# intel/intel-extension-for-transformers

Measured on AMD Instinct MI355X. Metric: decode tokens/sec + achieved HBM GB/s, Llama-2-7B int4 WOQ, batch=1, higher is better.
Workload: dtype int4 weights x fp32 activations (3 int8 limbs on i8 MFMA, exact int32 tile sums, fp32 across tiles); 1 GPU; Llama-2-7B int4 sym group_size=128 fp16 scales, batch=1 greedy decode, prompt 32, lm_head fp16 unquantised, KV fp16; global_batch=1, parallelism=single GPU, hipgraph=True

## Files before the change

intel_extension_for_transformers_amd/csrc/woq_ops.hip:

```cpp
#include "woq_attn_decode.h"
#include "woq_device.h"
#include "woq_host.h"
#include "woq_xq.h"
#include "../../include/woq_hip_experimental.h"

namespace woq {

__global__ __launch_bounds__(256) void rmsnorm_kernel(const void* __restrict__ x, int dtype,
                                                      const float* __restrict__ w, float eps, int d,
                                                      void* __restrict__ out, int out_dtype) {
  __shared__ float part[4];
  const size_t row = blockIdx.x;
  const int tid = threadIdx.x;
  float ss = 0.f;
  for (int i = tid; i < d; i += 256) {
    float v = load_f32(x, row * d + i, dtype);
    ss = fmaf(v, v, ss);
  }
  ss = wave_sum(ss);
  if ((tid & 63) == 0) part[tid >> 6] = ss;
  __syncthreads();
  const float tot = part[0] + part[1] + part[2] + part[3];
  const float inv = 1.0f / sqrtf(tot / (float)d + eps);
  for (int i = tid; i < d; i += 256) {
    float v = load_f32(x, row * d + i, dtype);
    store_f32(out, row * d + i, out_dtype, v * inv * w[i]);
  }
}

__global__ void rope_kernel(void* __restrict__ x, int dtype, const int32_t* __restrict__ pos,
                            const float* __restrict__ cs, const float* __restrict__ sn, int heads, int D,
                            size_t total_pairs) {
  size_t idx = (size_t)blockIdx.x * blockDim.x + threadIdx.x;
  if (idx >= total_pairs) return;
  const int half = D >> 1;
  const int i = (int)(idx % half);
  const size_t th = idx / half;
  const int t = (int)(th / heads);
  const int p = pos[t];
  const float c = cs[(size_t)p * half + i], s = sn[(size_t)p * half + i];
  const size_t base = th * D;
  const float a = load_f32(x, base + i, dtype), b = load_f32(x, base + i + half, dtype);
  store_f32(x, base + i, dtype, a * c - b * s);
  store_f32(x, base + i + half, dtype, b * c + a * s);
}

__global__ void silu_mul_kernel(const void* __restrict__ g, const void* __restrict__ u, int dtype, size_t n,
                                void* __restrict__ out) {
  size_t idx = (size_t)blockIdx.x * blockDim.x + threadIdx.x;
  const size_t stride = (size_t)gridDim.x * blockDim.x;
  for (; idx < n; idx += stride) {
    const float a = load_f32(g, idx, dtype), b = load_f32(u, idx, dtype);
    store_f32(out, idx, dtype, a / (1.0f + expf(-a)) * b);
  }
}

__global__ void gelu_kernel(const void* __restrict__ x, int dtype, size_t n, int approximate,
                            void* __restrict__ out) {
  size_t idx = (size_t)blockIdx.x * blockDim.x + threadIdx.x;
  const size_t stride = (size_t)gridDim.x * blockDim.x;
  for (; idx < n; idx += stride) {
    const float v = load_f32(x, idx, dtype);
    float r;
    if (approximate)
      r = 0.5f * v * (1.0f + tanhf(0.7978845608028654f * (v + 0.044715f * v * v * v)));
    else
      r = 0.5f * v * (1.0f + erff(v * 0.7071067811865476f));
    store_f32(out, idx, dtype, r);
  }
}


__global__ void embed_kernel(const void* __restrict__ embed, int dtype, const int32_t* __restrict__ token, int hidden,
                             float* __restrict__ out, const float* __restrict__ norm_w, XqPtrs xo,
                             float* __restrict__ ssq_out, unsigned int* __restrict__ step_seq,
                             int32_t* __restrict__ pos, int max_ctx, int* __restrict__ status) {
  const int i = blockIdx.x * blockDim.x + threadIdx.x;
  if (i == 0) {
    if (step_seq != nullptr) step_seq[0] = step_seq[0] + 1u;
    if (pos != nullptr && pos[0] >= max_ctx) {
      pos[0] = max_ctx - 1;
      if (status != nullptr) atomicOr(status, 2);
    }
  }
  if (i < hidden) {
    const float v = load_f32(embed, (size_t)token[0] * hidden + i, dtype);
    out[i] = v;
    if (xo.limbs != nullptr) {
      const float ss = row16_sum(v * v);
      if ((i & 15) == 0) ssq_out[i >> 4] = ss;
      xq_emit16(v * norm_w[i], xo, i >> 4, i & 15);
    }
  }
}

__global__ __launch_bounds__(256) void argmax_embed_kernel(const float* __restrict__ pmax, const int32_t* __restrict__ pidx,
                                                           int n_pairs, int32_t* __restrict__ token,
                                                           int32_t* __restrict__ pos, int32_t* __restrict__ log,
                                                           const void* __restrict__ embed, int dtype, int hidden,
                                                           float* __restrict__ out, const float* __restrict__ norm_w,
                                                           XqPtrs xo, float* __restrict__ ssq_out,
                                                           unsigned int* __restrict__ step_seq, int max_ctx,
                                                           int* __restrict__ status) {
  __shared__ float bv[4];
  __shared__ int bi[4];
  const int tid = threadIdx.x, lane = tid & 63, wid = tid >> 6;
  float best = -INFINITY;
  int idx = 0x7fffffff;
  for (int i = tid; i < n_pairs; i += 256) {
    const float v = pmax[i];
    const int ci = pidx[i];
    if (v > best || (v == best && ci < idx)) best = v, idx = ci;
  }
#pragma unroll
  for (int o = 32; o > 0; o >>= 1) {
    const float ov = __shfl_xor(best, o, 64);
    const int oi = __shfl_xor(idx, o, 64);
    if (ov > best || (ov == best && oi < idx)) best = ov, idx = oi;
  }
  if (lane == 0) bv[wid] = best, bi[wid] = idx;
  __syncthreads();
  best = bv[0], idx = bi[0];
#pragma unroll
  for (int w = 1; w < 4; ++w)
    if (bv[w] > best || (bv[w] == best && bi[w] < idx)) best = bv[w], idx = bi[w];
  const bool no_winner = idx < 0 || (size_t)idx >= (size_t)n_pairs * 16;
  if (no_winner) idx = 0;
  if (blockIdx.x == 0 && tid == 0) {
    if (no_winner && status != nullptr) atomicOr(status, 4);
    token[0] = idx;
    int p = pos[0];
    if (log != nullptr) log[p] = idx;
    p += 1;
    if (step_seq != nullptr) step_seq[0] = step_seq[0] + 1u;
    if (p >= max_ctx) {
      p = max_ctx - 1;
      if (status != nullptr) atomicOr(status, 2);
    }
    pos[0] = p;
  }
  const int i = blockIdx.x * 256 + tid;
  if (i < hidden) {
    const float v = load_f32(embed, (size_t)idx * hidden + i, dtype);
    out[i] = v;
    if (xo.limbs != nullptr) {
      const float ss = row16_sum(v * v);
      if ((i & 15) == 0) ssq_out[i >> 4] = ss;
      xq_emit16(v * norm_w[i], xo, i >> 4, i & 15);
    }
  }
}

template <typename KV, int HD, bool SPLIT>
__global__ __launch_bounds__(256) void attn_decode_kernel(const float* __restrict__ qkv, KV* __restrict__ kcache,
                                                          KV* __restrict__ vcache, const int32_t* __restrict__ pos_p,
                                                          const float* __restrict__ cs, const float* __restrict__ sn,
                                                          int hk, int window, int spw,
                                                          float* __restrict__ out, XqPtrs xo, AttnMerge mg) {
  extern __shared__ __attribute__((aligned(16))) float sm[];
  const int heads = hk & 0xffff, kv_heads = hk >> 16;
  const int bx = (int)blockIdx.x;
  const int h = (heads & 7) == 0 ? (bx & 7) * (heads >> 3) + (bx >> 3) : bx;
  attn_decode_body<KV, HD, SPLIT>(sm, h, (int)blockIdx.y, (int)gridDim.y, AttnPlain{qkv}, kcache, vcache, pos_p, cs,
                                  sn, heads, kv_heads, window, spw, out, xo);
  if constexpr (SPLIT) {
    if (mg.counter != nullptr) attn_slices_merge<HD, 1>(out, heads, h, 1, (int)gridDim.y, mg.counter + h, mg, sm);
  }
}

template <int HD>
__global__ __launch_bounds__(256) void attn_combine_kernel(const float* __restrict__ part, int ns,
                                                          float* __restrict__ out, XqPtrs xo) {
  __shared__ float ms[64], wl[64], wsc[64], red[256];
  constexpr int GROUPS = 256 / HD;
  constexpr int PER = ATTN_MAX_SLICES / GROUPS;
  const int h = blockIdx.x, tid = threadIdx.x;
  const int d = tid % HD, grp = tid / HD;
  const float* p = part + (size_t)h * ATTN_MAX_SLICES * HD;
  const float* pml = part + (size_t)gridDim.x * ATTN_MAX_SLICES * HD + (size_t)h * ATTN_MAX_SLICES * 2;
  const int si = min(tid, ns - 1);
  const float m_r = pml[si * 2], l_r = pml[si * 2 + 1];
  float v[PER];
#pragma unroll
  for (int u = 0; u < PER; ++u) v[u] = p[(size_t)min(grp + u * GROUPS, ns - 1) * HD + d];
  if (tid < ns) ms[tid] = m_r, wl[tid] = l_r;
  __syncthreads();
  float m = -INFINITY;
  for (int s = 0; s < ns; ++s) m = fmaxf(m, ms[s]);
  if (tid < ns) {
    const float w = ms[tid] == -INFINITY ? 0.f : __expf(ms[tid] - m);
    wsc[tid] = w;
    wl[tid] *= w;
  }
  __syncthreads();
  float l = 0.f;
  for (int s = 0; s < ns; ++s) l += wl[s];
  float o = 0.f;
#pragma unroll
  for (int u = 0; u < PER; ++u) {
    const int s = grp + u * GROUPS;
    if (s < ns) o = fmaf(v[u], wsc[s], o);
  }
  red[tid] = o;
  __syncthreads();
  if (grp == 0) {
    float t = 0.f;
#pragma unroll
    for (int g2 = 0; g2 < GROUPS; ++g2) t += red[g2 * HD + d];
    out[(size_t)h * HD + d] = t / l;
    if (xo.limbs != nullptr) xq_emit16(t / l, xo, (h * HD + d) >> 4, d & 15);
  }
}

__global__ __launch_bounds__(256) void lm_head_kernel(const float* __restrict__ hidden_in,
                                                      const float* __restrict__ norm_w, float eps,
                                                      const void* __restrict__ W, int w_dtype, int hidden, int vocab,
                                                      float* __restrict__ logits, float* __restrict__ pmax,
                                                      int32_t* __restrict__ pidx) {
  extern __shared__ __attribute__((aligned(16))) float sm[];
  float* xs = sm;
  __shared__ float part[4];
  __shared__ float bestv[4];
  __shared__ int besti[4];
  const int tid = threadIdx.x, lane = tid & 63, wid = tid >> 6;
  float wbest = -INFINITY;
  int wbi = 0x7fffffff;
  typedef unsigned int u32x4 __attribute__((ext_vector_type(4)));
  float ss = 0.f;
  for (int i = tid; i < hidden; i += 256) {
    const float v = hidden_in[i];
    xs[i] = v;
    ss = fmaf(v, v, ss);
  }
  ss = wave_sum(ss);
  if (lane == 0) part[wid] = ss;
  __syncthreads();
  const float inv = 1.0f / sqrtf((part[0] + part[1] + part[2] + part[3]) / (float)hidden + eps);
  for (int i = tid; i < hidden; i += 256) xs[i] = xs[i] * inv * norm_w[i];
  __syncthreads();
  const int rows_per_wg = 16;
  auto consume = [&](const u32x4& raw, int k0, float& acc) {
    const uint32_t rr[4] = {raw.x, raw.y, raw.z, raw.w};
#pragma unroll
    for (int j = 0; j < 4; ++j) {
      float lo, hi;
      if (w_dtype == WOQ_BF16) {
        lo = bf16_bits_to_f32(rr[j] & 0xffff);
        hi = bf16_bits_to_f32(rr[j] >> 16);
      } else {
        lo = f16_bits_to_f32(rr[j] & 0xffff);
        hi = f16_bits_to_f32(rr[j] >> 16);
      }
      acc = fmaf(lo, xs[k0 + 2 * j], acc);
      acc = fmaf(hi, xs[k0 + 2 * j + 1], acc);
    }
  };
  auto finish = [&](int v, float acc) {
    acc = wave_sum(acc);
    if (lane == 0) logits[v] = acc;
    if (acc > wbest) {
      wbest = acc;
      wbi = v;
    }
  };
  for (int r = wid; r < rows_per_wg; r += 4) {
    const int v = blockIdx.x * rows_per_wg + r;
    if (v >= vocab) break;
    const uint16_t* wr = (const uint16_t*)W + (size_t)v * hidden;
    float acc = 0.f;
    for (int k0 = lane * 8; k0 < hidden; k0 += 512) consume(__builtin_nontemporal_load((const u32x4*)(wr + k0)), k0, acc);
    finish(v, acc);
  }
  if (pmax) {
    if (lane == 0) {
      bestv[wid] = wbest;
      besti[wid] = wbi;
    }
    __syncthreads();
    if (tid == 0) {
      float b = bestv[0];
      int bi = besti[0];
      for (int w = 1; w < 4; ++w)
        if (bestv[w] > b || (bestv[w] == b && besti[w] < bi)) {
          b = bestv[w];
          bi = besti[w];
        }
      pmax[blockIdx.x] = b;
      pidx[blockIdx.x] = bi;
    }
  }
}

__global__ __launch_bounds__(1024) void argmax_kernel(const float* __restrict__ logits, const int32_t* __restrict__ cand,
                                                      int vocab, int32_t* __restrict__ token,
                                                      int32_t* __restrict__ pos, int32_t* __restrict__ log) {
  __shared__ float bv[16];
  __shared__ int bi[16];
  const int tid = threadIdx.x, lane = tid & 63, wid = tid >> 6;
  float best = -INFINITY;
  int idx = 0x7fffffff;
  for (int i = tid; i < vocab; i += 1024) {
    const float v = logits[i];
    const int ci = cand ? cand[i] : i;
    if (v > best || (v == best && ci < idx)) {
      best = v;
      idx = ci;
    }
  }
#pragma unroll
  for (int o = 32; o > 0; o >>= 1) {
    const float ov = __shfl_xor(best, o, 64);
    const int oi = __shfl_xor(idx, o, 64);
    if (ov > best || (ov == best && oi < idx)) {
      best = ov;
      idx = oi;
    }
  }
  if (lane == 0) {
    bv[wid] = best;
    bi[wid] = idx;
  }
  __syncthreads();
  if (tid == 0) {
    for (int w = 1; w < 16; ++w)
      if (bv[w] > best || (bv[w] == best && bi[w] < idx)) {
        best = bv[w];
        idx = bi[w];
      }
    token[0] = idx;
    if (log != nullptr) log[pos[0]] = idx;
    pos[0] = pos[0] + 1;
  }
}

void launch_embed(const void* embed, int dtype, const int32_t* token, int hidden, float* out, const float* norm_w,
                  const XqPtrs& xo, float* ssq_out, unsigned int* step_seq, int32_t* pos, int max_ctx, int* status,
                  hipStream_t st) {
  hipLaunchKernelGGL(embed_kernel, dim3((hidden + 255) / 256), dim3(256), 0, st, embed, dtype, token, hidden, out,
                     norm_w, xo, ssq_out, step_seq, pos, max_ctx, status);
}

template <typename KV, int HD>
static int launch_attn_t(const float* qkv, void* kcache, void* vcache, const int32_t* pos, const float* cs,
                         const float* sn, int heads, int kv_heads, int max_ctx, int window, float* out, int splits,
                         float* part, const XqPtrs& xo, unsigned int* merge_counters, hipStream_t st) {
  const int reach = window > 0 ? min(window, max_ctx) : max_ctx;
  const int span = splits > 1 ? ((((reach + splits - 1) / splits) + 63) & ~63) + 64 : reach;
  const int spw = attn_dec_spw(span);
  const size_t lds = attn_dec_lds_floats(HD, span) * 4;
  if (lds > 160 * 1024) return woq::fail("QBits: max_ctx too large for the decode attention (raise attn_splits)");
  if (splits > 1) {
    auto k = attn_decode_kernel<KV, HD, true>;
    static bool once = false;
    if (!once) {
      hipFuncSetAttribute((const void*)k, hipFuncAttributeMaxDynamicSharedMemorySize, 160 * 1024);
      once = true;
    }
    const AttnMerge mg{merge_counters, out, xo};
    hipLaunchKernelGGL(k, dim3(heads, splits), dim3(256), lds, st, qkv, (KV*)kcache, (KV*)vcache, pos, cs, sn,
                       heads | (kv_heads << 16), window, spw, part, XqPtrs{nullptr, nullptr, nullptr}, mg);
    if (merge_counters == nullptr)
      hipLaunchKernelGGL(attn_combine_kernel<HD>, dim3(heads), dim3(256), 0, st, part, splits, out, xo);
    return 0;
  }
  auto k = attn_decode_kernel<KV, HD, false>;
  static bool once = false;
  if (!once) {
    hipFuncSetAttribute((const void*)k, hipFuncAttributeMaxDynamicSharedMemorySize, 160 * 1024);
    once = true;
  }
  hipLaunchKernelGGL(k, dim3(heads), dim3(256), lds, st, qkv, (KV*)kcache, (KV*)vcache, pos, cs, sn,
                     heads | (kv_heads << 16), window, spw, out, xo,
                     AttnMerge{nullptr, nullptr, XqPtrs{nullptr, nullptr, nullptr}});
  return 0;
}

int launch_attn_decode(const float* qkv, void* kcache, void* vcache, int kv_dtype, const int32_t* pos,
                       const float* cs, const float* sn, int heads, int kv_heads, int D, int max_ctx, int window,
                       float* out, int splits, int grouped, float* part, const XqPtrs& xo, hipStream_t st,
                       unsigned int* merge_counters, int chunk_fixed, const AttnA2A* a2a_grouped, const unsigned int* seq,
                       int layer) {
  if (D != 64 && D != 128) return woq::fail("QBits: attention head_dim must be 64 or 128");
  if (splits > ATTN_MAX_SLICES) return woq::fail("QBits: at most 64 context slices");
  AttnMerge mg{merge_counters, out, xo};
  const bool a2a = grouped && a2a_grouped != nullptr && merge_counters == nullptr && splits <= 32;
  if (a2a) mg.part_g = a2a_grouped->part_g, mg.seq = seq, mg.layer = layer, mg.status = a2a_grouped->status;
  if (grouped && launch_attn_decode_mfma(qkv, kcache, vcache, kv_dtype, pos, cs, sn, heads, kv_heads, D, window, splits,
                                          part, chunk_fixed, max_ctx, mg, st)) {
    if (merge_counters == nullptr && !a2a) launch_attn_combine(part, heads, D, splits, out, xo, st);
    return 0;
  }
#define WOQ_ATTN_DEC(T)                                                                                              \
  return D == 128 ? launch_attn_t<T, 128>(qkv, kcache, vcache, pos, cs, sn, heads, kv_heads, max_ctx, window, out,   \
                                          splits, part, xo, merge_counters, st)                                     \
                  : launch_attn_t<T, 64>(qkv, kcache, vcache, pos, cs, sn, heads, kv_heads, max_ctx, window, out,    \
                                         splits, part, xo, merge_counters, st);
  if (kv_dtype == WOQ_F16) { WOQ_ATTN_DEC(_Float16) }
  if (kv_dtype == WOQ_FP8_E4M3) { WOQ_ATTN_DEC(Fp8) }
  WOQ_ATTN_DEC(__bf16)
#undef WOQ_ATTN_DEC
}

void launch_attn_combine(const float* part, int heads, int D, int splits, float* out, const XqPtrs& xo,
                         hipStream_t st) {
  if (D == 128)
    hipLaunchKernelGGL(attn_combine_kernel<128>, dim3(heads), dim3(256), 0, st, part, splits, out, xo);
  else
    hipLaunchKernelGGL(attn_combine_kernel<64>, dim3(heads), dim3(256), 0, st, part, splits, out, xo);
}

void launch_lm_head(const float* hidden_in, const float* norm_w, float eps, const void* W, int w_dtype, int hidden,
                    int vocab, float* logits, float* pmax, int32_t* pidx, hipStream_t st) {
  hipLaunchKernelGGL(lm_head_kernel, dim3((vocab + 15) / 16), dim3(256), (size_t)hidden * 4, st, hidden_in, norm_w,
                     eps, W, w_dtype, hidden, vocab, logits, pmax, pidx);
}

void launch_argmax(const float* logits, int vocab, int32_t* token, int32_t* pos, hipStream_t st) {
  hipLaunchKernelGGL(argmax_kernel, dim3(1), dim3(1024), 0, st, logits, (const int32_t*)nullptr, vocab, token, pos,
                     (int32_t*)nullptr);
}

void launch_argmax_pairs(const float* pmax, const int32_t* pidx, int n, int32_t* token, int32_t* pos, int32_t* log,
                         hipStream_t st) {
  hipLaunchKernelGGL(argmax_kernel, dim3(1), dim3(1024), 0, st, pmax, pidx, n, token, pos, log);
}

void launch_argmax_embed(const float* pmax, const int32_t* pidx, int n, int32_t* token, int32_t* pos, int32_t* log,
                         const void* embed, int dtype, int hidden, float* out, const float* norm_w, const XqPtrs& xo,
                         float* ssq_out, unsigned int* step_seq, int max_ctx, int* status, hipStream_t st) {
  hipLaunchKernelGGL(argmax_embed_kernel, dim3((hidden + 255) / 256), dim3(256), 0, st, pmax, pidx, n, token, pos, log,
                     embed, dtype, hidden, out, norm_w, xo, ssq_out, step_seq, max_ctx, status);
}

}

using namespace woq;

extern "C" {

int woq_rmsnorm(const void* x_dev, int dtype, const float* weight_dev, float eps, int rows, int d, void* out_dev,
                int out_dtype, void* stream) {
  WOQ_TRY
  WOQ_CHECK(rows >= 0 && d > 0, "QBits: bad rmsnorm shape");
  if (rows == 0) return 0;
  hipLaunchKernelGGL(rmsnorm_kernel, dim3(rows), dim3(256), 0, (hipStream_t)stream, x_dev, dtype, weight_dev, eps, d,
                     out_dev, out_dtype);
  WOQ_HIP(hipGetLastError());
  WOQ_END
}

int woq_rope(void* x_dev, int dtype, const int32_t* pos_dev, const float* cos_dev, const float* sin_dev, int tokens,
             int heads, int D, void* stream) {
  WOQ_TRY
  WOQ_CHECK((D & 1) == 0, "QBits: rope head_dim must be even");
  size_t total = (size_t)tokens * heads * (D / 2);
  if (total == 0) return 0;
  hipLaunchKernelGGL(rope_kernel, dim3((unsigned)((total + 255) / 256)), dim3(256), 0, (hipStream_t)stream, x_dev,
                     dtype, pos_dev, cos_dev, sin_dev, heads, D, total);
  WOQ_HIP(hipGetLastError());
  WOQ_END
}

int woq_silu_mul(const void* gate_dev, const void* up_dev, int dtype, size_t n, void* out_dev, void* stream) {
  WOQ_TRY
  if (n == 0) return 0;
  unsigned blocks = (unsigned)std::min<size_t>((n + 255) / 256, 2048);
  hipLaunchKernelGGL(silu_mul_kernel, dim3(blocks), dim3(256), 0, (hipStream_t)stream, gate_dev, up_dev, dtype, n,
                     out_dev);
  WOQ_HIP(hipGetLastError());
  WOQ_END
}

int woq_gelu(const void* x_dev, int dtype, size_t n, int approximate, void* out_dev, void* stream) {
  WOQ_TRY
  if (n == 0) return 0;
  unsigned blocks = (unsigned)std::min<size_t>((n + 255) / 256, 2048);
  hipLaunchKernelGGL(gelu_kernel, dim3(blocks), dim3(256), 0, (hipStream_t)stream, x_dev, dtype, n, approximate,
                     out_dev);
  WOQ_HIP(hipGetLastError());
  WOQ_END
}

WOQ_API int woq_probe_attn_decode(const float* qkv, void* kcache, void* vcache, int kv_dtype, const int32_t* pos_dev,
                                  const float* cos_dev, const float* sin_dev, int heads, int kv_heads, int head_dim,
                                  int max_ctx, int window, int splits, int grouped, int merge, int chunk_fixed,
                                  float* out, void* stream) {
  WOQ_TRY
  WOQ_CHECK(heads > 0 && kv_heads > 0 && heads % kv_heads == 0 && max_ctx > 0 && window >= 0 && splits >= 1,
            "QBits: bad attention shape");
  WOQ_CHECK(merge == 0 || merge == 1, "QBits: merge must be 0 (combine launch) or 1 (last-arriver counters)");
  const hipStream_t st = (hipStream_t)stream;
  const size_t part_bytes = (size_t)heads * ATTN_MAX_SLICES * (head_dim + 2) * sizeof(float);
  float* part = nullptr;
  unsigned int* counters = nullptr;
  WOQ_HIP(hipMallocAsync((void**)&part, part_bytes, st));
  if (merge) {
    if (hipMallocAsync((void**)&counters, (size_t)heads * sizeof(unsigned int), st) != hipSuccess ||
        hipMemsetAsync(counters, 0, (size_t)heads * sizeof(unsigned int), st) != hipSuccess) {
      if (counters) hipFreeAsync(counters, st);
      hipFreeAsync(part, st);
      return woq::fail("QBits: could not allocate the attention merge counters");
    }
  }
  const int rc = launch_attn_decode(qkv, kcache, vcache, kv_dtype, pos_dev, cos_dev, sin_dev, heads, kv_heads, head_dim,
                                    max_ctx, window, out, splits, grouped, part, XqPtrs{nullptr, nullptr, nullptr}, st,
                                    counters, chunk_fixed, nullptr, nullptr, 0);
  const hipError_t le = hipGetLastError();
  if (counters) hipFreeAsync(counters, st);
  hipFreeAsync(part, st);
  if (rc) return rc;
  WOQ_HIP(le);
  WOQ_END
}

}
```

Before: 689.4 tokens/s.

## Software-pipeline lm_head weight streaming with buffer loads and templated chunk count

New measurement: 692.9 tokens/s (median of 6 runs). About the same (+0.5%).

```diff
diff --git a/intel_extension_for_transformers_amd/csrc/woq_lm_head.h b/intel_extension_for_transformers_amd/csrc/woq_lm_head.h
--- /dev/null
+++ b/intel_extension_for_transformers_amd/csrc/woq_lm_head.h
@@ -0,0 +1,192 @@
+#pragma once
+#include "woq_device.h"
+#include "woq_gemv_common.h"
+
+namespace woq {
+
+constexpr int LM_WINDOW = 8;
+constexpr int LM_EARLY = 0;
+
+template <bool BF, int CPR, int D, int EARLY>
+__device__ __forceinline__ void lm_head_stream(float* __restrict__ xs, float* __restrict__ part,
+                                               float* __restrict__ bestv, int* __restrict__ besti,
+                                               const float* __restrict__ hidden_in, const float* __restrict__ norm_w,
+                                               float eps, const void* __restrict__ W, int hidden, int vocab,
+                                               float* __restrict__ logits, float* __restrict__ pmax,
+                                               int32_t* __restrict__ pidx) {
+  const int tid = threadIdx.x, lane = tid & 63;
+  const int wid = __builtin_amdgcn_readfirstlane(tid >> 6);
+  const int row0 = (int)blockIdx.x * 16;
+  const int cpr = CPR > 0 ? CPR : (hidden + 511) >> 9;
+  const int total = 4 * cpr;
+  const int pitch = hidden * 2;
+  const rsrc_t rw = make_rsrc((const uint16_t*)W + (size_t)row0 * hidden, min(16, vocab - row0) * pitch);
+  const int lane8 = lane * 8;
+
+  int q_i = 0, q_off = wid * pitch;
+  int c_i = 0, c_row = row0 + wid;
+  u32x4 w[D];
+  auto request = [&](u32x4& dst) {
+    const int k0 = lane8 + (q_i << 9);
+    dst = __builtin_amdgcn_raw_buffer_load_b128(rw, k0 < hidden ? q_off + k0 * 2 : 0x7ffffff0, 0, AUX_NT);
+    if (++q_i == cpr) q_i = 0, q_off += 4 * pitch;
+  };
+  int q_base = wid * pitch + lane8 * 2;
+  auto request_at = [&](u32x4& dst, int c) {
+    const int i = c % cpr;
+    const int off = q_base + ((i & 3) << 10);
+    const bool live = i + 1 < cpr || lane8 + (i << 9) < hidden;
+    dst = __builtin_amdgcn_raw_buffer_load_b128(rw, live ? off : 0x7ffffff0, 0, AUX_NT);
+    if (i + 1 == cpr)
+      q_base += 4 * pitch - ((i >> 2) << 12);
+    else if ((i & 3) == 3)
+      q_base += 4096;
+    else
+      return;
+    asm volatile("" : "+v"(q_base));
+  };
+  auto fill = [&]() {
+#pragma unroll
+    for (int s = 0; s < D; ++s) {
+      if constexpr (CPR > 0) {
+        if (s < 4 * CPR) request_at(w[s], s);
+      } else {
+        if (s < total) request(w[s]);
+      }
+    }
+    __builtin_amdgcn_sched_barrier(0);
+  };
+
+  if constexpr (EARLY == 1) fill();
+  const rsrc_t rh = make_rsrc(hidden_in, hidden * 4), rn = make_rsrc(norm_w, hidden * 4);
+  float ss = 0.f;
+  for (int b = tid; b < hidden; b += 2048) {
+    float v[8];
+#pragma unroll
+    for (int u = 0; u < 8; ++u)
+      v[u] = __builtin_bit_cast(float, __builtin_amdgcn_raw_buffer_load_b32(rh, (b + 256 * u) * 4, 0, 0));
+#pragma unroll
+    for (int u = 0; u < 8; ++u)
+      if (b + 256 * u < hidden) {
+        xs[b + 256 * u] = v[u];
+        ss = fmaf(v[u], v[u], ss);
+      }
+  }
+  if constexpr (EARLY == 2) fill();
+  ss = wave_sum(ss);
+  if (lane == 0) part[wid] = ss;
+  __syncthreads();
+  const float inv = 1.0f / sqrtf((part[0] + part[1] + part[2] + part[3]) / (float)hidden + eps);
+  for (int b = tid; b < hidden; b += 2048) {
+    float g[8];
+#pragma unroll
+    for (int u = 0; u < 8; ++u)
+      g[u] = __builtin_bit_cast(float, __builtin_amdgcn_raw_buffer_load_b32(rn, (b + 256 * u) * 4, 0, 0));
+#pragma unroll
+    for (int u = 0; u < 8; ++u)
+      if (b + 256 * u < hidden) xs[b + 256 * u] = xs[b + 256 * u] * inv * g[u];
+  }
+  __syncthreads();
+  if constexpr (EARLY == 0) fill();
+
+  float wbest = -INFINITY;
+  int wbi = 0x7fffffff;
+  float acc = 0.f;
+  float mine = 0.f;
+  int c_j = 0;
+  auto fma8 = [&](const u32x4& raw, int k0, bool live) {
+    const int kc = live ? k0 : 0;
+    const float4_t x0 = *(const float4_t*)(xs + kc), x1 = *(const float4_t*)(xs + kc + 4);
+    const float x[8] = {x0.x, x0.y, x0.z, x0.w, x1.x, x1.y, x1.z, x1.w};
+    const uint32_t rr[4] = {raw.x, raw.y, raw.z, raw.w};
+    float t = acc;
+#pragma unroll
+    for (int j = 0; j < 4; ++j) {
+      float lo, hi;
+      if constexpr (BF) {
+        lo = bf16_bits_to_f32(rr[j] & 0xffff);
+        hi = bf16_bits_to_f32(rr[j] >> 16);
+      } else {
+        lo = f16_bits_to_f32(rr[j] & 0xffff);
+        hi = f16_bits_to_f32(rr[j] >> 16);
+      }
+      t = fmaf(lo, x[2 * j], t);
+      t = fmaf(hi, x[2 * j + 1], t);
+    }
+    acc = live ? t : acc;
+  };
+  auto consume = [&](const u32x4& raw) {
+    const int k0 = lane8 + (c_i << 9);
+    fma8(raw, k0, k0 < hidden);
+    if (++c_i == cpr) {
+      if (c_row < vocab) {
+        const float sum = wave_sum(acc);
+        mine = lane == c_j ? sum : mine;
+        if (sum > wbest) wbest = sum, wbi = c_row;
+      }
+      c_i = 0, c_row += 4, c_j += 1, acc = 0.f;
+    }
+  };
+
+  if constexpr (CPR > 0) {
+    constexpr int TOTAL = 4 * CPR;
+#pragma unroll
+    for (int c = 0; c < TOTAL; ++c) {
+      const int k0 = lane8 + ((c % CPR) << 9);
+      fma8(w[c % D], k0, (c % CPR) + 1 < CPR || k0 < hidden);
+      if (c + D < TOTAL) request_at(w[c % D], c + D);
+      if ((c % CPR) + 1 == CPR) {
+        const int row = row0 + wid + 4 * (c / CPR);
+        const float sum = wave_sum(acc);
+        mine = lane == c / CPR ? sum : mine;
+        if (row < vocab && sum > wbest) wbest = sum, wbi = row;
+        acc = 0.f;
+      }
+      __builtin_amdgcn_sched_barrier(0x38f);
+    }
+  } else {
+  int c = 0;
+  for (; c + 2 * D <= total; c += D) {
+#pragma unroll
+    for (int s = 0; s < D; ++s) {
+      consume(w[s]);
+      request(w[s]);
+      __builtin_amdgcn_sched_barrier(0x38f);
+    }
+  }
+  const int rem = total - c;
+#pragma unroll
+  for (int s = 0; s < D; ++s) {
+    if (s < rem) {
+      consume(w[s]);
+      if (s + D < rem) request(w[s]);
+    }
+    __builtin_amdgcn_sched_barrier(0x38f);
+  }
+#pragma unroll
+  for (int s = 0; s < D; ++s)
+    if (s + D < rem) consume(w[s]);
+  }
+  if (lane < 4 && row0 + wid + 4 * lane < vocab) logits[row0 + wid + 4 * lane] = mine;
+
+  if (pmax) {
+    if (lane == 0) {
+      bestv[wid] = wbest;
+      besti[wid] = wbi;
+    }
+    __syncthreads();
+    if (tid == 0) {
+      float b = bestv[0];
+      int bi = besti[0];
+      for (int w2 = 1; w2 < 4; ++w2)
+        if (bestv[w2] > b || (bestv[w2] == b && besti[w2] < bi)) {
+          b = bestv[w2];
+          bi = besti[w2];
+        }
+      pmax[blockIdx.x] = b;
+      pidx[blockIdx.x] = bi;
+    }
+  }
+}
+
+}
diff --git a/intel_extension_for_transformers_amd/csrc/woq_ops.hip b/intel_extension_for_transformers_amd/csrc/woq_ops.hip
--- a/intel_extension_for_transformers_amd/csrc/woq_ops.hip
+++ b/intel_extension_for_transformers_amd/csrc/woq_ops.hip
@@ -1,6 +1,7 @@
 #include "woq_attn_decode.h"
 #include "woq_device.h"
 #include "woq_host.h"
+#include "woq_lm_head.h"
 #include "woq_xq.h"
 #include "../../include/woq_hip_experimental.h"
 
@@ -212,83 +213,21 @@
   }
 }
 
-__global__ __launch_bounds__(256) void lm_head_kernel(const float* __restrict__ hidden_in,
-                                                      const float* __restrict__ norm_w, float eps,
-                                                      const void* __restrict__ W, int w_dtype, int hidden, int vocab,
-                                                      float* __restrict__ logits, float* __restrict__ pmax,
-                                                      int32_t* __restrict__ pidx) {
+template <int CPR>
+__global__ __launch_bounds__(256) __attribute__((amdgpu_waves_per_eu(8, 8))) void lm_head_kernel(
+    const float* __restrict__ hidden_in, const float* __restrict__ norm_w, float eps, const void* __restrict__ W,
+    int w_dtype, int hidden, int vocab, float* __restrict__ logits, float* __restrict__ pmax,
+    int32_t* __restrict__ pidx) {
   extern __shared__ __attribute__((aligned(16))) float sm[];
-  float* xs = sm;
   __shared__ float part[4];
   __shared__ float bestv[4];
   __shared__ int besti[4];
-  const int tid = threadIdx.x, lane = tid & 63, wid = tid >> 6;
-  float wbest = -INFINITY;
-  int wbi = 0x7fffffff;
-  typedef unsigned int u32x4 __attribute__((ext_vector_type(4)));
-  float ss = 0.f;
-  for (int i = tid; i < hidden; i += 256) {
-    const float v = hidden_in[i];
-    xs[i] = v;
-    ss = fmaf(v, v, ss);
-  }
-  ss = wave_sum(ss);
-  if (lane == 0) part[wid] = ss;
-  __syncthreads();
-  const float inv = 1.0f / sqrtf((part[0] + part[1] + part[2] + part[3]) / (float)hidden + eps);
-  for (int i = tid; i < hidden; i += 256) xs[i] = xs[i] * inv * norm_w[i];
-  __syncthreads();
-  const int rows_per_wg = 16;
-  auto consume = [&](const u32x4& raw, int k0, float& acc) {
-    const uint32_t rr[4] = {raw.x, raw.y, raw.z, raw.w};
-#pragma unroll
-    for (int j = 0; j < 4; ++j) {
-      float lo, hi;
-      if (w_dtype == WOQ_BF16) {
-        lo = bf16_bits_to_f32(rr[j] & 0xffff);
-        hi = bf16_bits_to_f32(rr[j] >> 16);
-      } else {
-        lo = f16_bits_to_f32(rr[j] & 0xffff);
-        hi = f16_bits_to_f32(rr[j] >> 16);
-      }
-      acc = fmaf(lo, xs[k0 + 2 * j], acc);
-      acc = fmaf(hi, xs[k0 + 2 * j + 1], acc);
-    }
-  };
-  auto finish = [&](int v, float acc) {
-    acc = wave_sum(acc);
-    if (lane == 0) logits[v] = acc;
-    if (acc > wbest) {
-      wbest = acc;
-      wbi = v;
-    }
-  };
-  for (int r = wid; r < rows_per_wg; r += 4) {
-    const int v = blockIdx.x * rows_per_wg + r;
-    if (v >= vocab) break;
-    const uint16_t* wr = (const uint16_t*)W + (size_t)v * hidden;
-    float acc = 0.f;
-    for (int k0 = lane * 8; k0 < hidden; k0 += 512) consume(__builtin_nontemporal_load((const u32x4*)(wr + k0)), k0, acc);
-    finish(v, acc);
-  }
-  if (pmax) {
-    if (lane == 0) {
-      bestv[wid] = wbest;
-      besti[wid] = wbi;
-    }
-    __syncthreads();
-    if (tid == 0) {
-      float b = bestv[0];
-      int bi = besti[0];
-      for (int w = 1; w < 4; ++w)
-        if (bestv[w] > b || (bestv[w] == b && besti[w] < bi)) {
-          b = bestv[w];
-          bi = besti[w];
-        }
-      pmax[blockIdx.x] = b;
-      pidx[blockIdx.x] = bi;
-    }
-  }
+  if (w_dtype == WOQ_BF16)
+    lm_head_stream<true, CPR, LM_WINDOW, LM_EARLY>(sm, part, bestv, besti, hidden_in, norm_w, eps, W, hidden, vocab,
+                                                   logits, pmax, pidx);
+  else
+    lm_head_stream<false, CPR, LM_WINDOW, LM_EARLY>(sm, part, bestv, besti, hidden_in, norm_w, eps, W, hidden, vocab,
+                                                    logits, pmax, pidx);
 }
 
 __global__ __launch_bounds__(1024) void argmax_kernel(const float* __restrict__ logits, const int32_t* __restrict__ cand,
@@ -411,8 +350,15 @@
 
 void launch_lm_head(const float* hidden_in, const float* norm_w, float eps, const void* W, int w_dtype, int hidden,
                     int vocab, float* logits, float* pmax, int32_t* pidx, hipStream_t st) {
-  hipLaunchKernelGGL(lm_head_kernel, dim3((vocab + 15) / 16), dim3(256), (size_t)hidden * 4, st, hidden_in, norm_w,
-                     eps, W, w_dtype, hidden, vocab, logits, pmax, pidx);
+  auto k = lm_head_kernel<0>;
+  switch ((hidden + 511) / 512) {
+    case 1: k = lm_head_kernel<1>; break;
+    case 2: k = lm_head_kernel<2>; break;
+    case 4: k = lm_head_kernel<4>; break;
+    case 8: k = lm_head_kernel<8>; break;
+  }
+  hipLaunchKernelGGL(k, dim3((vocab + 15) / 16), dim3(256), (size_t)hidden * 4, st, hidden_in, norm_w, eps, W, w_dtype,
+                     hidden, vocab, logits, pmax, pidx);
 }
 
 void launch_argmax(const float* logits, int vocab, int32_t* token, int32_t* pos, hipStream_t st) {
```
